# jack-nie/bitcoin-miner

Hardware: AMD Instinct MI355X
Metric: GH/s (SHA-256 nonce search) at 1/2/4/8 MI355X; % of VALU int roofline (higher is better)
Workload: dtype u32

## Files before the change

### bitcoin-miner_amd/csrc/minehip.cpp

```cpp
#include <hip/hip_runtime.h>
#include <stdlib.h>
#include <string.h>

#include <atomic>
#include <chrono>
#include <cmath>
#include <condition_variable>
#include <memory>
#include <mutex>
#include <string>
#include <system_error>
#include <thread>
#include <vector>

#include "../../include/minehip.h"
#include "../../include/minehip_server.h"
#include "layout.hpp"
#include "multi.hpp"
#include "plan.hpp"
#include "sched.hpp"

namespace mh {
hipError_t fast_module_init(int dev);
hipError_t launch_fast(int dev, int J, int mode, const FastArgs& a, Partial* partials, hipStream_t s);
hipError_t launch_generic_scan(const GenArgs& a, Partial* partials, uint32_t blocks, hipStream_t s);
hipError_t launch_hash_batch(const GenArgs& a, const uint64_t* d_nonces, uint64_t* d_out, uint64_t n,
                             hipStream_t s);
hipError_t launch_merge(const Partial* partials, uint32_t n, Partial* best, hipStream_t s);
}

namespace {

using mh::Partial;

thread_local std::string g_err;

int fail(int code, const std::string& what) {
    g_err = what;
    return code;
}

}

namespace mh {
int set_error(int code, const char* what) { return fail(code, what); }
}

namespace {

#define MH_HIP(call)                                                                                 \
    do {                                                                                             \
        hipError_t e_ = (call);                                                                      \
        if (e_ != hipSuccess) return fail(MH_EHIP, std::string(#call) + ": " + hipGetErrorString(e_)); \
    } while (0)

constexpr uint64_t kBatchChunk = 1u << 22;
constexpr int kEventPairs = 512;
constexpr uint32_t kQueueSlots = 4096;

struct Timed {
    hipEvent_t start = nullptr, stop = nullptr;
    int kind;
    int var;
};

struct VarStat {
    uint64_t launches = 0, nonces = 0, ns = 0, ops = 0, slots = 0;
};
constexpr int kVariants = 16 * mh::kModes * 5;
inline int var_index(int J, int mode, int L) { return J + 16 * mode + 16 * mh::kModes * (L - 1); }

struct DevCtx {
    std::mutex mu;
    int dev = -1;
    bool ready = false;
    hipStream_t stream = nullptr;
    hipStream_t ps[2] = {nullptr, nullptr};
    hipEvent_t ev_piece[2] = {nullptr, nullptr};
    hipEvent_t ev_main = nullptr;
    Partial* d_partials = nullptr;
    Partial* d_best = nullptr;
    Partial* h_best = nullptr;
    uint64_t* d_nonces = nullptr;
    uint64_t* d_hashes = nullptr;
    uint32_t poff = 0;
    uint32_t* d_counters = nullptr;
    uint32_t qoff = 0;
    bool prof = false;
    std::vector<Timed> pool;
    int used = 0;
    uint64_t cnt[8] = {0};
    VarStat var[kVariants];
};

std::mutex g_tab_mu;
std::vector<std::unique_ptr<DevCtx>> g_tab;
int g_ndev = -1;

int device_count_impl() {
    std::lock_guard<std::mutex> lk(g_tab_mu);
    if (g_ndev < 0) {
        int n = 0;
        if (hipGetDeviceCount(&n) != hipSuccess) n = 0;
        g_ndev = n;
        g_tab.resize((size_t)n);
        for (auto& p : g_tab) p.reset(new DevCtx());
    }
    return g_ndev;
}

int get_ctx(int dev, DevCtx** out) {
    const int n = device_count_impl();
    if (n <= 0) return fail(MH_ENODEV, "no HIP device visible");
    if (dev < 0 || dev >= n) return fail(MH_EINVAL, "device index out of range");
    DevCtx* c = g_tab[(size_t)dev].get();
    *out = c;
    return MH_OK;
}

int init_locked(DevCtx* c, int dev) {
    if (c->ready) return MH_OK;
    MH_HIP(hipSetDevice(dev));
    hipDeviceProp_t prop;
    MH_HIP(hipGetDeviceProperties(&prop, dev));
    if (strncmp(prop.gcnArchName, "gfx950", 6) != 0)
        return fail(MH_ENODEV, std::string("device is ") + prop.gcnArchName + ", kernels are built for gfx950 only");
    if (!c->stream) MH_HIP(hipStreamCreateWithFlags(&c->stream, hipStreamNonBlocking));
    if (!c->ps[0] || !c->ps[1]) {
        int least = 0, greatest = 0;
        MH_HIP(hipDeviceGetStreamPriorityRange(&least, &greatest));
        if (!c->ps[0]) MH_HIP(hipStreamCreateWithPriority(&c->ps[0], hipStreamNonBlocking, greatest));
        if (!c->ps[1]) MH_HIP(hipStreamCreateWithPriority(&c->ps[1], hipStreamNonBlocking, least));
    }
    for (auto& e : c->ev_piece)
        if (!e) MH_HIP(hipEventCreateWithFlags(&e, hipEventDisableTiming));
    if (!c->ev_main) MH_HIP(hipEventCreateWithFlags(&c->ev_main, hipEventDisableTiming));
    if (!c->d_partials) MH_HIP(hipMalloc(&c->d_partials, sizeof(Partial) * mh::kMaxBlocksPerLaunch));
    if (!c->d_best) MH_HIP(hipMalloc(&c->d_best, sizeof(Partial)));
    if (!c->d_counters) MH_HIP(hipMalloc(&c->d_counters, sizeof(uint32_t) * kQueueSlots));
    if (!c->h_best) MH_HIP(hipHostMalloc(&c->h_best, sizeof(Partial), hipHostMallocDefault));
    if (!c->d_nonces) MH_HIP(hipMalloc(&c->d_nonces, sizeof(uint64_t) * kBatchChunk));
    if (!c->d_hashes) MH_HIP(hipMalloc(&c->d_hashes, sizeof(uint64_t) * kBatchChunk));
    if (c->pool.empty()) c->pool.resize(kEventPairs);
    for (auto& t : c->pool) {
        if (!t.start) MH_HIP(hipEventCreate(&t.start));
        if (!t.stop) MH_HIP(hipEventCreate(&t.stop));
    }
    MH_HIP(mh::fast_module_init(dev));
    c->dev = dev;
    c->ready = true;
    return MH_OK;
}

int harvest_locked(DevCtx* c) {
    for (int i = 0; i < c->used; ++i) {
        float ms = 0.f;
        MH_HIP(hipEventElapsedTime(&ms, c->pool[(size_t)i].start, c->pool[(size_t)i].stop));
        const uint64_t ns = (uint64_t)((double)ms * 1.0e6);
        c->cnt[c->pool[(size_t)i].kind == 0 ? 2 : 5] += ns;
        if (c->pool[(size_t)i].kind == 0) c->var[c->pool[(size_t)i].var].ns += ns;
    }
    c->used = 0;
    return MH_OK;
}

int piece_streams_wait_main(DevCtx* c) {
    MH_HIP(hipEventRecord(c->ev_main, c->stream));
    for (auto s : c->ps) MH_HIP(hipStreamWaitEvent(s, c->ev_main, 0));
    return MH_OK;
}

int flush_partials(DevCtx* c, bool split) {
    if (!c->poff) return MH_OK;
    if (split) {
        for (int k = 0; k < 2; ++k) {
            MH_HIP(hipEventRecord(c->ev_piece[k], c->ps[k]));
            MH_HIP(hipStreamWaitEvent(c->stream, c->ev_piece[k], 0));
        }
    }
    MH_HIP(mh::launch_merge(c->d_partials, c->poff, c->d_best, c->stream));
    c->poff = 0;
    if (split) return piece_streams_wait_main(c);
    return MH_OK;
}

bool coarse_piece(const mh::Piece& p, const mh::PlanOpts& opt) { return p.kind == 0 && p.L == opt.lower_digits; }

bool early_piece_ok(const mh::Piece& p) {
    const mh::FastArgs& a = p.fa;
    const uint32_t J = (uint32_t)p.J;
    if ((a.inner >> 2) != J || a.hole + a.hole_w > a.n_hi + a.L) return false;
    for (uint32_t j = 0; j + 1u < a.L; ++j) {
        const uint32_t pos = a.g_last - j - (j >= a.g_hole ? 1u : 0u);
        if (pos > a.g_last || (pos >> 2) != J) return false;
    }
    return true;
}

int enqueue_piece(DevCtx* c, const mh::Piece& p, const mh::PlanOpts& opt, bool split) {
    hipStream_t s = !split ? c->stream : c->ps[coarse_piece(p, opt) ? 0 : 1];
    uint32_t blocks;
    if (p.kind == 0) {
        if (p.fa.n_runs == 0 || p.fa.L < 1 || p.fa.L > 5 || p.fa.n_hi + p.fa.L > 20)
            return fail(MH_EINTERNAL, "internal: bad fast piece");
        if (p.fa.mode >= mh::kModeOneEarly && !early_piece_ok(p))
            return fail(MH_EINTERNAL, "internal: bad Early piece (an enumerated digit outside word J)");
        blocks = (p.fa.n_runs + mh::kBlockThreads - 1) / mh::kBlockThreads;
    } else {
        if (p.ga.count == 0 || p.ga.count > (uint64_t)mh::kMaxBlocksPerLaunch * mh::kBlockThreads)
            return fail(MH_EINTERNAL, "internal: bad generic piece");
        blocks = (uint32_t)((p.ga.count + mh::kBlockThreads - 1) / mh::kBlockThreads);
    }
    if (blocks > mh::kMaxBlocksPerLaunch) return fail(MH_EINTERNAL, "internal: grid too large");
    if (c->poff + blocks > mh::kMaxBlocksPerLaunch) {
        const int rc = flush_partials(c, split);
        if (rc) return rc;
    }
    Partial* out = c->d_partials + c->poff;
    Timed* tm = nullptr;
    mh::FastArgs fa = p.fa;
    if (p.kind == 0) {
        fa.n_chunks = blocks;
        fa.counter = (opt.queue && c->qoff < kQueueSlots) ? c->d_counters + c->qoff++ : nullptr;
    }
    if (c->prof) {
        if (c->used == kEventPairs) {
            MH_HIP(hipStreamSynchronize(c->stream));
            for (auto ps : c->ps) MH_HIP(hipStreamSynchronize(ps));
            int rc = harvest_locked(c);
            if (rc) return rc;
        }
        tm = &c->pool[(size_t)c->used++];
        tm->kind = p.kind;
        tm->var = p.kind == 0 ? var_index(p.J, p.mode, p.L) : 0;
        MH_HIP(hipEventRecord(tm->start, s));
    }
    if (p.kind == 0)
        MH_HIP(mh::launch_fast(c->dev, p.J, p.mode, fa, out, s));
    else
        MH_HIP(mh::launch_generic_scan(p.ga, out, blocks, s));
    if (tm) MH_HIP(hipEventRecord(tm->stop, s));
    c->poff += blocks;
    if (c->prof) {
        if (p.kind == 0) {
            const uint64_t n = p.count;
            c->cnt[0] += 1;
            c->cnt[1] += n;
            c->cnt[3] += n * (uint64_t)p.ops;
            c->cnt[6] += n * (uint64_t)p.slots;
            VarStat& v = c->var[var_index(p.J, p.mode, p.L)];
            v.launches += 1;
            v.nonces += n;
            v.ops += n * (uint64_t)p.ops;
            v.slots += n * (uint64_t)p.slots;
        } else {
            c->cnt[4] += p.count;
        }
    }
    return MH_OK;
}

mh::PlanOpts plan_opts() {
    mh::PlanOpts o;
    if (const char* e = getenv("MINEHIP_LOWER_DIGITS")) {
        const int v = atoi(e);
        if (v >= 1 && v <= 5) o.lower_digits = v;
    }
    if (const char* e = getenv("MINEHIP_MIN_LANES")) o.min_lanes = strtoull(e, nullptr, 10);
    if (const char* e = getenv("MINEHIP_LAUNCH_NONCES")) {
        const unsigned long long v = strtoull(e, nullptr, 10);
        if (v >= 1) o.max_nonces_per_launch = v;
    }
    if (const char* e = getenv("MINEHIP_GENERIC_BELOW")) o.generic_below = strtoull(e, nullptr, 10);
    if (const char* e = getenv("MINEHIP_MAX_BLOCKS")) {
        const unsigned long long v = strtoull(e, nullptr, 10);
        if (v >= 1 && v <= mh::kMaxBlocksPerLaunch) o.max_blocks = (uint32_t)v;
    }
    if (const char* e = getenv("MINEHIP_STREAMS")) {
        const int v = atoi(e);
        if (v == 1 || v == 2) o.streams = v;
    }
    if (const char* e = getenv("MINEHIP_FINE_TAIL")) o.fine_tail = strtoull(e, nullptr, 10);
    if (const char* e = getenv("MINEHIP_QUEUE")) {
        const int v = atoi(e);
        if (v == 0 || v == 1) o.queue = v;
    }
    if (const char* e = getenv("MINEHIP_EARLY")) {
        const int v = atoi(e);
        if (v == 0 || v == 1) o.early = v;
    }
    return o;
}

uint64_t now_ns() {
    return (uint64_t)std::chrono::duration_cast<std::chrono::nanoseconds>(
               std::chrono::steady_clock::now().time_since_epoch())
        .count();
}

int search_impl(int dev, const mh::Prefix& pre, uint64_t lower, uint64_t upper, uint64_t* oh, uint64_t* on,
                uint64_t* busy_ns = nullptr) {
    DevCtx* c;
    int rc = get_ctx(dev, &c);
    if (rc) return rc;
    std::lock_guard<std::mutex> lk(c->mu);
    rc = init_locked(c, dev);
    if (rc) return rc;
    const uint64_t t0 = now_ns();
    MH_HIP(hipSetDevice(dev));
    MH_HIP(hipMemsetAsync(c->d_best, 0xFF, sizeof(Partial), c->stream));
    const mh::PlanOpts opt = plan_opts();
    if (opt.queue) MH_HIP(hipMemsetAsync(c->d_counters, 0, sizeof(uint32_t) * kQueueSlots, c->stream));
    c->qoff = 0;
    bool any_coarse = false, any_fine = false;
    if (opt.streams == 2)
        mh::plan_search(pre, lower, upper, opt, [&](const mh::Piece& p) {
            (coarse_piece(p, opt) ? any_coarse : any_fine) = true;
            return !(any_coarse && any_fine);
        });
    const bool split = opt.streams == 2 && any_coarse && any_fine;
    if (split) {
        rc = piece_streams_wait_main(c);
        if (rc) return rc;
    }
    int err = MH_OK;
    c->poff = 0;
    mh::plan_search(pre, lower, upper, opt, [&](const mh::Piece& p) {
        err = enqueue_piece(c, p, opt, split);
        return err == MH_OK;
    });
    if (!err) err = flush_partials(c, split);
    if (err) {
        for (auto ps : c->ps)
            if (ps) (void)hipStreamSynchronize(ps);
        (void)hipStreamSynchronize(c->stream);
        return err;
    }
    MH_HIP(hipMemcpyAsync(c->h_best, c->d_best, sizeof(Partial), hipMemcpyDeviceToHost, c->stream));
    MH_HIP(hipStreamSynchronize(c->stream));
    if (c->prof) {
        rc = harvest_locked(c);
        if (rc) return rc;
    }
    *oh = c->h_best->hash;
    *on = c->h_best->nonce;
    if (busy_ns) *busy_ns = now_ns() - t0;
    return MH_OK;
}

int check_common(const uint8_t* msg, size_t len) {
    if (msg == nullptr && len != 0) return fail(MH_EINVAL, "msg is NULL");
    if (len > MH_MAX_MSG_LEN) return fail(MH_ETOOLONG, "message longer than MH_MAX_MSG_LEN");
    return MH_OK;
}

}

extern "C" {

int mh_abi_version(void) { return MH_ABI_VERSION; }

int mh_device_count(void) { return device_count_impl(); }

const char* mh_last_error(void) { return g_err.c_str(); }

int mh_search(int dev, const uint8_t* msg, size_t len, uint64_t lower, uint64_t upper, uint64_t* out_hash,
              uint64_t* out_nonce) {
    g_err.clear();
    if (!out_hash || !out_nonce) return fail(MH_EINVAL, "NULL output pointer");
    int rc = check_common(msg, len);
    if (rc) return rc;
    if (lower > upper) return fail(MH_ERANGE, "lower > upper");
    mh::Prefix pre;
    mh::absorb_prefix(msg, len, &pre);
    return search_impl(dev, pre, lower, upper, out_hash, out_nonce);
}

int mh_search_multi(const int* devs, int ndev, const uint8_t* msg, size_t len, uint64_t lower, uint64_t upper,
                    uint64_t chunk, uint64_t* out_hash, uint64_t* out_nonce) {
    g_err.clear();
    if (!out_hash || !out_nonce || !devs || ndev <= 0) return fail(MH_EINVAL, "bad arguments");
    if (ndev > MH_MAX_WORKERS) return fail(MH_EINVAL, "more than MH_MAX_WORKERS devices listed");
    int rc = check_common(msg, len);
    if (rc) return rc;
    if (lower > upper) return fail(MH_ERANGE, "lower > upper");
    const int n = mh_device_count();
    for (int i = 0; i < ndev; ++i)
        if (devs[i] < 0 || devs[i] >= n) return fail(n <= 0 ? MH_ENODEV : MH_EINVAL, "device index out of range");
    mh::Prefix pre;
    mh::absorb_prefix(msg, len, &pre);
    int fail_worker = -1;
    mh::ThreadStart start;
#ifdef MH_DEV_HOOKS
    if (const char* e = getenv("MINEHIP_TEST_FAIL_WORKER")) fail_worker = atoi(e);
    if (const char* e = getenv("MINEHIP_TEST_SPAWN_LIMIT")) {
        auto started = std::make_shared<std::atomic<int>>(0);
        const int limit = atoi(e);
        start = [started, limit](std::function<void()> fn) {
            if ((*started)++ >= limit)
                throw std::system_error(std::make_error_code(std::errc::resource_unavailable_try_again));
            return std::thread(std::move(fn));
        };
    }
#endif
    if (ndev == 1 && chunk == 0 && fail_worker < 0 && !start)
        return search_impl(devs[0], pre, lower, upper, out_hash, out_nonce);
    if (chunk == 0) {
        const mh::SpanSearch search = [&](int worker, int dev, uint64_t lo, uint64_t hi, uint64_t* h, uint64_t* n,
                                          uint64_t* ns, std::string* err) {
            const int r = (worker == fail_worker) ? fail(MH_EHIP, "injected failure (dev build test hook)")
                                                  : search_impl(dev, pre, lo, hi, h, n, ns);
            if (r) *err = g_err;
            return r;
        };
        std::string err;
        const int r = mh::search_shards(devs, ndev, pre, lower, upper, plan_opts(), search, out_hash, out_nonce, &err,
                                        start);
        return r ? fail(r, err) : MH_OK;
    }
    const mh::ChunkSearch csearch = [&](int worker, uint64_t lo, uint64_t hi, uint64_t* h, uint64_t* nn,
                                        std::string* err) {
        const int r = (worker == fail_worker) ? fail(MH_EHIP, "injected failure (dev build test hook)")
                                              : search_impl(devs[worker], pre, lo, hi, h, nn);
        if (r) *err = g_err;
        return r;
    };
    std::string err;
    const int r = mh::search_chunks(ndev, msg, len, lower, upper, chunk, csearch, out_hash, out_nonce, &err, start);
    return r ? fail(r, err) : MH_OK;
}

int mh_hash_batch(int dev, const uint8_t* msg, size_t len, const uint64_t* nonces, size_t n, uint64_t* out_hashes) {
    g_err.clear();
    int rc = check_common(msg, len);
    if (rc) return rc;
    if (n == 0) return MH_OK;
    if (!nonces || !out_hashes) return fail(MH_EINVAL, "NULL buffer");
    DevCtx* c;
    rc = get_ctx(dev, &c);
    if (rc) return rc;
    std::lock_guard<std::mutex> lk(c->mu);
    rc = init_locked(c, dev);
    if (rc) return rc;
    MH_HIP(hipSetDevice(dev));
    mh::Prefix pre;
    mh::absorb_prefix(msg, len, &pre);
    mh::GenArgs ga;
    mh::make_gen_args(pre, &ga);
    for (size_t off = 0; off < n; off += kBatchChunk) {
        const size_t m = (n - off < kBatchChunk) ? n - off : kBatchChunk;
        MH_HIP(hipMemcpyAsync(c->d_nonces, nonces + off, m * sizeof(uint64_t), hipMemcpyHostToDevice, c->stream));
        MH_HIP(mh::launch_hash_batch(ga, c->d_nonces, c->d_hashes, m, c->stream));
        MH_HIP(hipMemcpyAsync(out_hashes + off, c->d_hashes, m * sizeof(uint64_t), hipMemcpyDeviceToHost, c->stream));
        MH_HIP(hipStreamSynchronize(c->stream));
    }
    return MH_OK;
}

int mh_profile_enable(int dev, int on) {
    g_err.clear();
    DevCtx* c;
    int rc = get_ctx(dev, &c);
    if (rc) return rc;
    std::lock_guard<std::mutex> lk(c->mu);
    rc = init_locked(c, dev);
    if (rc) return rc;
    MH_HIP(hipStreamSynchronize(c->stream));
    rc = harvest_locked(c);
    if (rc) return rc;
    if (on) {
        memset(c->cnt, 0, sizeof c->cnt);
        for (auto& v : c->var) v = VarStat();
    }
    c->prof = on != 0;
    return MH_OK;
}

int mh_profile_read(int dev, uint64_t* out, int n) {
    g_err.clear();
    if (!out || n < 0) return fail(MH_EINVAL, "bad arguments");
    DevCtx* c;
    int rc = get_ctx(dev, &c);
    if (rc) return rc;
    std::lock_guard<std::mutex> lk(c->mu);
    if (c->ready) {
        MH_HIP(hipStreamSynchronize(c->stream));
        rc = harvest_locked(c);
        if (rc) return rc;
    }
    for (int i = 0; i < n && i < 8; ++i) out[i] = c->cnt[i];
    return MH_OK;
}

int mh_profile_kernels(int dev, mh_kernel_stat* out, int cap) {
    g_err.clear();
    if (cap < 0 || (!out && cap > 0)) return fail(MH_EINVAL, "bad arguments");
    DevCtx* c;
    int rc = get_ctx(dev, &c);
    if (rc) return rc;
    std::lock_guard<std::mutex> lk(c->mu);
    if (c->ready) {
        MH_HIP(hipStreamSynchronize(c->stream));
        rc = harvest_locked(c);
        if (rc) return rc;
    }
    int n = 0;
    for (int i = 0; i < kVariants; ++i) {
        const VarStat& v = c->var[i];
        if (!v.launches) continue;
        if (n < cap) {
            out[n].word = i % 16;
            out[n].mode = (i / 16) % mh::kModes;
            out[n].lo_digits = i / (16 * mh::kModes) + 1;
            out[n].reserved = 0;
            out[n].launches = v.launches;
            out[n].nonces = v.nonces;
            out[n].ns = v.ns;
            out[n].ops = v.ops;
            out[n].slots = v.slots;
        }
        ++n;
    }
    return n;
}

int64_t mh_plan(const uint8_t* msg, size_t len, uint64_t lower, uint64_t upper, mh_piece* out, int64_t cap) {
    g_err.clear();
    int rc = check_common(msg, len);
    if (rc) return rc;
    if (lower > upper) return fail(MH_ERANGE, "lower > upper");
    if (cap < 0) return fail(MH_EINVAL, "cap < 0");
    mh::Prefix pre;
    mh::absorb_prefix(msg, len, &pre);
    int64_t k = 0;
    const mh::PlanOpts opt = plan_opts();
    mh::plan_search(pre, lower, upper, opt, [&](const mh::Piece& p) {
        if (k >= cap) {
            ++k;
            return false;
        }
        if (out) {
            mh_piece& q = out[k];
            q.first = p.first;
            q.count = p.count;
            q.kind = p.kind;
            q.digits = p.digits;
            q.lo_digits = p.L;
            q.word = p.J;
            q.mode = p.mode;
            q.blocks = p.blocks;
            q.nonce_ops = p.ops;
            q.nonce_slots = p.slots;
        }
        ++k;
        return true;
    });
    return k;
}

int64_t mh_multi_plan(const uint8_t* msg, size_t len, uint64_t lower, uint64_t upper, const double* weights,
                      int ndev, mh_span* out, int64_t cap) {
    g_err.clear();
    int rc = check_common(msg, len);
    if (rc) return rc;
    if (lower > upper) return fail(MH_ERANGE, "lower > upper");
    if (ndev <= 0 || ndev > MH_MAX_WORKERS || cap < 0) return fail(MH_EINVAL, "bad arguments");
    std::vector<double> w((size_t)ndev, 1.0);
    if (weights)
        for (int i = 0; i < ndev; ++i) {
            if (!(weights[i] > 0.0) || !std::isfinite(weights[i])) return fail(MH_EINVAL, "weights must be finite and > 0");
            w[(size_t)i] = weights[i];
        }
    mh::Prefix pre;
    mh::absorb_prefix(msg, len, &pre);
    mh::MultiPlan mp;
    mh::multi_plan(pre, lower, upper, plan_opts(), w, &mp);
    int64_t k = 0;
    auto put = [&](const mh::Span& s, int worker, int kind) {
        if (k < cap && out) {
            out[k].lower = s.lo;
            out[k].upper = s.hi;
            out[k].worker = worker;
            out[k].kind = kind;
            out[k].cost = mh::segments_cost(mp.segs, s.lo, s.hi);
        }
        ++k;
    };
    for (int i = 0; i < ndev; ++i)
        if (!mp.head[(size_t)i].empty) put(mp.head[(size_t)i], i, 0);
    for (const auto& s : mp.tail) put(s, -1, 1);
    return k;
}

int mh_multi_rates(const int* devs, int ndev, double* out) {
    g_err.clear();
    if (ndev < 0 || (ndev > 0 && (!devs || !out))) return fail(MH_EINVAL, "bad arguments");
    for (int i = 0; i < ndev; ++i) out[i] = mh::device_rate(devs[i]);
    return MH_OK;
}

}
```

### bitcoin-miner_amd/csrc/plan.cpp

```cpp
#include "plan.hpp"

#include <string.h>

#include <algorithm>
#include <cmath>

namespace mh {
namespace {

constexpr uint32_t kK[64] = {
    0x428a2f98u, 0x71374491u, 0xb5c0fbcfu, 0xe9b5dba5u, 0x3956c25bu, 0x59f111f1u, 0x923f82a4u, 0xab1c5ed5u,
    0xd807aa98u, 0x12835b01u, 0x243185beu, 0x550c7dc3u, 0x72be5d74u, 0x80deb1feu, 0x9bdc06a7u, 0xc19bf174u,
    0xe49b69c1u, 0xefbe4786u, 0x0fc19dc6u, 0x240ca1ccu, 0x2de92c6fu, 0x4a7484aau, 0x5cb0a9dcu, 0x76f988dau,
    0x983e5152u, 0xa831c66du, 0xb00327c8u, 0xbf597fc7u, 0xc6e00bf3u, 0xd5a79147u, 0x06ca6351u, 0x14292967u,
    0x27b70a85u, 0x2e1b2138u, 0x4d2c6dfcu, 0x53380d13u, 0x650a7354u, 0x766a0abbu, 0x81c2c92eu, 0x92722c85u,
    0xa2bfe8a1u, 0xa81a664bu, 0xc24b8b70u, 0xc76c51a3u, 0xd192e819u, 0xd6990624u, 0xf40e3585u, 0x106aa070u,
    0x19a4c116u, 0x1e376c08u, 0x2748774cu, 0x34b0bcb5u, 0x391c0cb3u, 0x4ed8aa4au, 0x5b9cca4fu, 0x682e6ff3u,
    0x748f82eeu, 0x78a5636fu, 0x84c87814u, 0x8cc70208u, 0x90befffau, 0xa4506cebu, 0xbef9a3f7u, 0xc67178f2u};
constexpr uint32_t kIV[8] = {0x6a09e667u, 0xbb67ae85u, 0x3c6ef372u, 0xa54ff53au,
                             0x510e527fu, 0x9b05688cu, 0x1f83d9abu, 0x5be0cd19u};

inline uint32_t ror(uint32_t x, int n) { return (x >> n) | (x << (32 - n)); }

constexpr uint64_t kPow10[20] = {1ull,
                                 10ull,
                                 100ull,
                                 1000ull,
                                 10000ull,
                                 100000ull,
                                 1000000ull,
                                 10000000ull,
                                 100000000ull,
                                 1000000000ull,
                                 10000000000ull,
                                 100000000000ull,
                                 1000000000000ull,
                                 10000000000000ull,
                                 100000000000000ull,
                                 1000000000000000ull,
                                 10000000000000000ull,
                                 100000000000000000ull,
                                 1000000000000000000ull,
                                 10000000000000000000ull};

inline void put_byte(uint32_t* w, uint32_t pos, uint32_t v) { w[pos >> 2] |= v << (24u - 8u * (pos & 3u)); }

void schedule(const uint32_t w16[16], uint32_t w[64]) {
    for (int i = 0; i < 16; ++i) w[i] = w16[i];
    for (int i = 16; i < 64; ++i) {
        const uint32_t s0 = ror(w[i - 15], 7) ^ ror(w[i - 15], 18) ^ (w[i - 15] >> 3);
        const uint32_t s1 = ror(w[i - 2], 17) ^ ror(w[i - 2], 19) ^ (w[i - 2] >> 10);
        w[i] = w[i - 16] + s0 + w[i - 7] + s1;
    }
}

}

int decimal_digits(uint64_t n) {
    int d = 1;
    while (d < 20 && n >= kPow10[d]) ++d;
    return d;
}

void host_compress(uint32_t st[8], const uint32_t w16[16]) {
    uint32_t w[64];
    schedule(w16, w);
    uint32_t a = st[0], b = st[1], c = st[2], d = st[3], e = st[4], f = st[5], g = st[6], h = st[7];
    for (int i = 0; i < 64; ++i) {
        const uint32_t t1 = h + (ror(e, 6) ^ ror(e, 11) ^ ror(e, 25)) + ((e & f) ^ (~e & g)) + kK[i] + w[i];
        const uint32_t t2 = (ror(a, 2) ^ ror(a, 13) ^ ror(a, 22)) + ((a & b) ^ (a & c) ^ (b & c));
        h = g; g = f; f = e; e = d + t1;
        d = c; c = b; b = a; a = t1 + t2;
    }
    st[0] += a; st[1] += b; st[2] += c; st[3] += d;
    st[4] += e; st[5] += f; st[6] += g; st[7] += h;
}

void absorb_prefix(const uint8_t* msg, size_t len, Prefix* out) {
    memcpy(out->mid, kIV, sizeof kIV);
    out->plen = (uint64_t)len + 1u;
    const uint64_t nfull = out->plen / 64u;
    uint32_t w[16];
    for (uint64_t blk = 0; blk < nfull; ++blk) {
        for (int i = 0; i < 16; ++i) {
            uint32_t v = 0;
            for (int k = 0; k < 4; ++k) {
                const uint64_t p = blk * 64u + (uint64_t)(4 * i + k);
                const uint32_t byte = (p < len) ? msg[p] : (uint32_t)' ';
                v = (v << 8) | byte;
            }
            w[i] = v;
        }
        host_compress(out->mid, w);
    }
    out->t = (uint32_t)(out->plen % 64u);
    memset(out->tail, 0, sizeof out->tail);
    for (uint32_t i = 0; i < out->t; ++i) {
        const uint64_t p = nfull * 64u + i;
        out->tail[i] = (p < len) ? msg[p] : (uint8_t)' ';
    }
}

void make_gen_args(const Prefix& pre, GenArgs* ga) {
    memset(ga, 0, sizeof *ga);
    memcpy(ga->mid, pre.mid, sizeof pre.mid);
    for (uint32_t i = 0; i < pre.t; ++i) put_byte(ga->tail, i, pre.tail[i]);
    ga->plen = pre.plen;
    ga->t = pre.t;
}

NonceCost nonce_cost(int J, int mode) {
    uint64_t dep = 1ull << J;
    for (int t = 16; t < 64; ++t)
        if (((dep >> (t - 2)) | (dep >> (t - 7)) | (dep >> (t - 15)) | (dep >> (t - 16))) & 1ull) dep |= 1ull << t;
    auto is = [&](int t) { return (dep >> t) & 1ull; };
    uint32_t ops = 0, slots = 0;
    for (int t = 16; t < 64; ++t) {
        if (!is(t)) continue;
        const int s0 = (int)is(t - 15), s1 = (int)is(t - 2), a16 = (int)is(t - 16), a7 = (int)is(t - 7);
        const int hoisted = (s0 && s1 && a16 && a7) ? 0 : 1;
        const int terms = s0 + s1 + a16 + a7 + hoisted;
        const bool x0 = s0 && t - 15 == J, x1 = s1 && t - 2 == J;
        ops += (uint32_t)((s0 ? (x0 ? 1 : 4) : 0) + (s1 ? (x1 ? 1 : 4) : 0)) + (uint32_t)terms / 2u;
        slots += (uint32_t)((s0 ? (x0 ? 1 : 6) : 0) + (s1 ? (x1 ? 1 : 6) : 0)) + (uint32_t)(terms - 1);
    }
    ops += 3u;
    slots += 3u;
    for (int t = J + 1; t < 64; ++t) {
        const bool inv_w = !is(t), inv_h = inv_w && t <= J + 3;
        ops += inv_h ? 13u : 14u;
        slots += 16u + (inv_h ? 5u : inv_w ? 6u : 7u);
    }
    if (mode % 3 == kModeTwo) {
        ops += 8u;
        slots += 8u;
        ops += 64u * 14u - 1u;
        slots += 64u * 22u - 1u;
    } else {
        ops -= 1u;
        slots -= 1u;
    }
    ops += 2u;
    slots += 2u;
    return NonceCost{ops, slots};
}

uint32_t nonce_ops(int J, int mode) { return nonce_cost(J, mode).ops; }

namespace {

bool kernel_exists(int J, int mode) { return fast_kernel_exists(J, mode); }

bool make_fast_args(const Prefix& pre, int d, int L, bool early, int* J_out, int* mode_out, int* blocks_out,
                    uint64_t* block_out, FastArgs* fa) {
    const uint32_t t = pre.t;
    const uint32_t total = t + (uint32_t)d;
    const int nb = (total + 9u <= 64u) ? 1 : 2;
    const uint32_t pl = total - 1u;
    int mode;
    uint32_t base;
    if (nb == 1) {
        mode = kModeOne;
        base = 0;
    } else if (pl >= 64u) {
        mode = kModePre;
        base = 64;
        if (!early && pl - (uint32_t)L + 1u < 64u) return false;
    } else {
        mode = kModeTwo;
        base = 0;
    }
    const uint32_t lo = pl - (uint32_t)L + 1u - base;
    int J = (int)((pl - base) >> 2);
    uint32_t p = 0, ib = 0;
    if (!early) {
        if ((int)(lo >> 2) < J - 1) return false;
    } else {
        if (J < 1) return false;
        ib = base + 4u * (uint32_t)J - 1u;
        if (ib < t || ib < base) return false;
        p = pl - ib;
        if (p < 1u || p >= (uint32_t)d) return false;
        if (L > 4 || p + (uint32_t)L > (uint32_t)d || ib - (uint32_t)(L - 1) < t || ib - (uint32_t)(L - 1) < base)
            return false;
        J -= 1;
        mode += 3;
    }
    if (!kernel_exists(J, mode)) return false;

    memset(fa, 0, sizeof *fa);
    memcpy(fa->mid, pre.mid, sizeof pre.mid);
    for (uint32_t i = 0; i < t; ++i) put_byte(fa->blk, i, pre.tail[i]);
    for (uint32_t i = 0; i < (uint32_t)d; ++i) put_byte(fa->blk, t + i, 0x30u);
    put_byte(fa->blk, total, 0x80u);
    const uint64_t bits = (pre.plen + (uint64_t)d) * 8u;
    const int lw = nb * 16 - 2;
    fa->blk[lw] = (uint32_t)(bits >> 32);
    fa->blk[lw + 1] = (uint32_t)bits;
    fa->pow10L = kPow10[L];
    fa->hi_end = total - (uint32_t)L;
    fa->n_hi = (uint32_t)(d - L);
    fa->lo_pos = lo;
    fa->L = (uint32_t)L;
    fa->n_groups = (uint32_t)kPow10[L - 1];
    fa->mode = (uint32_t)mode;
    fa->hole = kNoHole;
    fa->g_hole = kNoHole;
    fa->hole_w = 1;
    fa->g_mul = 1;
    uint64_t block = kPow10[L];
    if (early) {
        fa->inner = ib - base;
        fa->i_mul = kPow10[p];
        fa->g_last = ib - 1u - base;
        fa->hi_end = total;
        fa->hole = p;
        fa->hole_w = (uint32_t)L;
        fa->u_mul = 1;
        fa->g_mul = kPow10[p + 1u];
        block = kPow10[p + (uint32_t)L];
    }
    *block_out = block;
    if (mode % 3 == kModeTwo) {
        uint32_t w[64];
        schedule(fa->blk + 16, w);
        for (int i = 0; i < 64; ++i) fa->kw1[i] = kK[i] + w[i];
    }
    *J_out = J;
    *mode_out = mode;
    *blocks_out = nb;
    return true;
}

bool pick_layout(const Prefix& pre, int d, int L, uint64_t A, uint64_t B, const PlanOpts& opt, int* J, int* mode,
                 int* nb, uint64_t* block, FastArgs* fa) {
    if (!make_fast_args(pre, d, L, false, J, mode, nb, block, fa)) return false;
    if (opt.early) {
        int Je, me, nbe;
        uint64_t be;
        FastArgs fe;
        const uint64_t max_gen = (uint64_t)std::min(opt.max_blocks, kMaxBlocksPerLaunch) * kBlockThreads;
        if (make_fast_args(pre, d, L, true, &Je, &me, &nbe, &be, &fe) &&
            nonce_cost(Je, me).slots < nonce_cost(*J, *mode).slots && B - A >= 2u * be &&
            be <= opt.max_nonces_per_launch && be / kPow10[L] <= max_gen) {
            *J = Je;
            *mode = me;
            *nb = nbe;
            *block = be;
            *fa = fe;
        }
    }
    return true;
}

bool bucket_layout(const Prefix& pre, int d, uint64_t A, uint64_t B, const PlanOpts& opt, int* L_out, int* J,
                   int* mode, int* nb, uint64_t* block, FastArgs* fa) {
    int L = std::min(opt.lower_digits, d - 1);
    L = std::min(L, 5);
    while (L > 1 && (B - A) / kPow10[L] + 1u < opt.min_lanes) --L;
    while (L >= 1 && !pick_layout(pre, d, L, A, B, opt, J, mode, nb, block, fa)) --L;
    *L_out = L;
    return L >= 1 && B - A >= opt.generic_below;
}

inline uint64_t bucket_lo(int d) { return d == 1 ? 0u : kPow10[d - 1]; }
inline uint64_t bucket_hi(int d) { return d == 20 ? ~(uint64_t)0 : kPow10[d] - 1u; }

}

void cost_segments(const Prefix& pre, uint64_t lower, uint64_t upper, const PlanOpts& opt,
                   std::vector<CostSeg>* out) {
    out->clear();
    const int d_lo = decimal_digits(lower), d_hi = decimal_digits(upper);
    for (int d = d_lo; d <= d_hi; ++d) {
        const uint64_t A = std::max(lower, bucket_lo(d)), B = std::min(upper, bucket_hi(d));
        int L = 0, J = 0, mode = 0, nb = 1;
        uint64_t blk = 1;
        FastArgs fa;
        double per;
        bool steady = false;
        if (bucket_layout(pre, d, A, B, opt, &L, &J, &mode, &nb, &blk, &fa)) {
            steady = L == opt.lower_digits && (B - A) / kPow10[L] + 1u >= (1u << 21);
            per = (double)nonce_cost(J, mode).slots * (1.0 + 0.03 * (double)(3 - std::min(L, 3)));
            if (!steady) per *= kUnsteadyFactor;
        } else {
            const int blocks = (pre.t + (uint32_t)d + 9u <= 64u) ? 1 : 2;
            per = (double)kGenericSlotsPerBlock * blocks;
        }
        out->push_back(CostSeg{A, B, per, steady});
    }
}

double unsteady_share(const std::vector<CostSeg>& segs, uint64_t lo, uint64_t hi) {
    double all = 0.0, unsteady = 0.0;
    for (const CostSeg& s : segs) {
        const uint64_t a = std::max(s.a, lo), b = std::min(s.b, hi);
        if (a > b) continue;
        const double c = ((double)(b - a) + 1.0) * s.per;
        all += c;
        if (!s.steady) unsteady += c;
    }
    return all > 0.0 ? unsteady / all : 0.0;
}

double segments_cost(const std::vector<CostSeg>& segs, uint64_t lo, uint64_t hi) {
    double c = 0.0;
    for (const CostSeg& s : segs) {
        const uint64_t a = std::max(s.a, lo), b = std::min(s.b, hi);
        if (a <= b) c += ((double)(b - a) + 1.0) * s.per;
    }
    return c;
}

void split_by_cost(const std::vector<CostSeg>& segs, const std::vector<double>& w, std::vector<Span>* out) {
    out->assign(w.size(), Span{0, 0, true});
    if (segs.empty() || w.empty()) return;
    using u128 = unsigned __int128;
    double wsum = 0.0;
    for (double x : w) wsum += std::max(0.0, x);
    double total = 0.0;
    for (const CostSeg& s : segs) total += ((double)(s.b - s.a) + 1.0) * s.per;
    const uint64_t lower = segs.front().a;
    const u128 n_all = (u128)(segs.back().b - lower) + 1u;
    u128 prev = 0;
    double acc_w = 0.0;
    for (size_t k = 0; k < w.size(); ++k) {
        acc_w += std::max(0.0, w[k]);
        u128 pos;
        if (k + 1 == w.size() || wsum <= 0.0) {
            pos = (k + 1 == w.size()) ? n_all : prev;
        } else {
            double target = total * (acc_w / wsum), cum = 0.0;
            pos = n_all;
            for (const CostSeg& s : segs) {
                const double len = (double)(s.b - s.a) + 1.0, c = len * s.per;
                if (cum + c >= target) {
                    double n = std::floor((target - cum) / s.per);
                    n = std::min(std::max(n, 0.0), len);
                    pos = (u128)(s.a - lower) + (u128)n;
                    break;
                }
                cum += c;
            }
            if (pos > n_all) pos = n_all;
        }
        if (pos < prev) pos = prev;
        if (pos > prev) (*out)[k] = Span{(uint64_t)(lower + (prev)), (uint64_t)(lower + (pos - 1u)), false};
        prev = pos;
    }
}

void plan_search(const Prefix& pre, uint64_t lower, uint64_t upper, const PlanOpts& opt,
                 const std::function<bool(const Piece&)>& cb) {
    GenArgs gbase;
    make_gen_args(pre, &gbase);
    const int d_lo = decimal_digits(lower), d_hi = decimal_digits(upper);
    const uint64_t max_gen = (uint64_t)std::min(opt.max_blocks, kMaxBlocksPerLaunch) * kBlockThreads;

    bool have_gen = false;
    uint64_t gen_a = 0, gen_b = 0;
    auto flush_generic = [&]() -> bool {
        if (!have_gen) return true;
        have_gen = false;
        Piece p;
        memset(&p, 0, sizeof p);
        p.first = gen_a;
        p.count = gen_b - gen_a + 1u;
        p.kind = 1;
        p.digits = decimal_digits(gen_a);
        p.blocks = ((pre.t + (uint32_t)decimal_digits(gen_b) + 9u) <= 64u) ? 1 : 2;
        p.ga = gbase;
        p.ga.first = gen_a;
        p.ga.count = p.count;
        return cb(p);
    };
    auto emit_generic = [&](uint64_t a, uint64_t b, int) -> bool {
        for (;;) {
            if (have_gen && gen_b - gen_a < max_gen - 1u && gen_b + 1u == a) {
                const uint64_t room = max_gen - 1u - (gen_b - gen_a);
                if (b - a < room) {
                    gen_b = b;
                    return true;
                }
                gen_b = a + (room - 1u);
                a = gen_b + 1u;
            }
            if (!flush_generic()) return false;
            const uint64_t left = b - a;
            const uint64_t cnt = (left >= max_gen - 1u) ? max_gen : left + 1u;
            have_gen = true;
            gen_a = a;
            gen_b = a + (cnt - 1u);
            if (cnt - 1u == left) return true;
            a += cnt;
        }
    };

    auto emit_runs = [&](int d, unsigned __int128 ua, unsigned __int128 ub, uint64_t Bx, int Lx, int Jx, int modex,
                         int nbx, const FastArgs& fax) -> bool {
        const unsigned __int128 Rx = kPow10[Lx];
        const uint64_t lpb = Bx / (uint64_t)Rx;
        uint64_t max_runs = std::min<uint64_t>(max_gen, opt.max_nonces_per_launch / (uint64_t)Rx);
        max_runs = std::max<uint64_t>(lpb, max_runs / lpb * lpb);
        ua *= lpb;
        ub *= lpb;
        for (unsigned __int128 u = ua; u < ub;) {
            const unsigned __int128 left = ub - u;
            const uint64_t runs = (left > max_runs) ? max_runs : (uint64_t)left;
            Piece p;
            memset(&p, 0, sizeof p);
            p.first = (uint64_t)(u * Rx);
            p.count = (uint64_t)((unsigned __int128)runs * Rx);
            p.kind = 0;
            p.digits = d;
            p.L = Lx;
            p.J = Jx;
            p.mode = modex;
            p.blocks = nbx;
            p.fa = fax;
            { const NonceCost nc = nonce_cost(Jx, modex); p.ops = nc.ops; p.slots = nc.slots; }
            p.fa.u_start = (uint64_t)u;
            p.fa.n_runs = (uint32_t)runs;
            p.ga = gbase;
            if (!flush_generic() || !cb(p)) return false;
            u += runs;
        }
        return true;
    };
    auto emit_edge = [&](int d, uint64_t a, uint64_t b) -> bool {
        FastArgs fs;
        int Js = 0, ms = 0, nbs = 1;
        uint64_t bs = 1;
        const int L = 1;
        if (!make_fast_args(pre, d, L, false, &Js, &ms, &nbs, &bs, &fs)) return emit_generic(a, b, d);
        const unsigned __int128 R = bs;
        const unsigned __int128 u0 = ((unsigned __int128)a + R - 1u) / R, u1 = ((unsigned __int128)b + 1u) / R;
        if (u0 >= u1) return emit_generic(a, b, d);
        if (a < (uint64_t)(u0 * R) && !emit_generic(a, (uint64_t)(u0 * R) - 1u, d)) return false;
        if (!emit_runs(d, u0, u1, bs, L, Js, ms, nbs, fs)) return false;
        return u1 * R > (unsigned __int128)b || emit_generic((uint64_t)(u1 * R), b, d);
    };

    for (int d = d_lo; d <= d_hi; ++d) {
        const uint64_t A = std::max(lower, bucket_lo(d)), B = std::min(upper, bucket_hi(d));
        FastArgs fa;
        int L = 0, J = 0, mode = 0, nb = 1;
        uint64_t blk = 1;
        if (!bucket_layout(pre, d, A, B, opt, &L, &J, &mode, &nb, &blk, &fa)) {
            if (!emit_generic(A, B, d)) return;
            continue;
        }
        const bool early = mode >= 3;
        const unsigned __int128 R = blk;
        const unsigned __int128 U0 = ((unsigned __int128)A + R - 1u) / R;
        const unsigned __int128 U1p = ((unsigned __int128)B + 1u) / R;
        if (U0 >= U1p) {
            if (!(early ? emit_edge(d, A, B) : emit_generic(A, B, d))) return;
            continue;
        }
        const uint64_t fast_first = (uint64_t)(U0 * R);
        const unsigned __int128 fast_end = U1p * R;
        if (A < fast_first && !(early ? emit_edge(d, A, fast_first - 1u) : emit_generic(A, fast_first - 1u, d)))
            return;
        unsigned __int128 U_split = U1p;
        int Lf = 0, Jf = 0, modef = 0, nbf = 1;
        uint64_t blkf = 1;
        FastArgs faf;
        if (opt.fine_tail && L == opt.lower_digits && L >= 2) {
            const unsigned __int128 tail_blocks = opt.fine_tail / (uint64_t)R;
            if (tail_blocks >= 1 && (U1p - U0) > 4 * tail_blocks &&
                pick_layout(pre, d, L - 1, A, B, opt, &Jf, &modef, &nbf, &blkf, &faf) && R % blkf == 0u) {
                U_split = U1p - tail_blocks;
                Lf = L - 1;
            }
        }
        if (!emit_runs(d, U0, U_split, blk, L, J, mode, nb, fa)) return;
        if (U_split < U1p && !emit_runs(d, U_split * (R / blkf), U1p * (R / blkf), blkf, Lf, Jf, modef, nbf, faf))
            return;
        if (fast_end <= (unsigned __int128)B &&
            !(early ? emit_edge(d, (uint64_t)fast_end, B) : emit_generic((uint64_t)fast_end, B, d)))
            return;
    }
    flush_generic();
}

}
```

### bitcoin-miner_amd/csrc/plan.hpp

```cpp
#pragma once
#include <stdint.h>
#include <stddef.h>

#include <functional>
#include <vector>

#include "layout.hpp"

namespace mh {

struct Prefix {
    uint32_t mid[8];
    uint8_t tail[64];
    uint32_t t;
    uint64_t plen;
};

void absorb_prefix(const uint8_t* msg, size_t len, Prefix* out);

void host_compress(uint32_t st[8], const uint32_t w16[16]);

struct Piece {
    uint64_t first;
    uint64_t count;
    int kind;
    int digits;
    int L;
    int J;
    int mode;
    int blocks;
    uint32_t ops;
    uint32_t slots;
    FastArgs fa;
    GenArgs ga;
};

struct PlanOpts {
    int lower_digits = 3;
    uint64_t min_lanes = 1u << 19;
    uint64_t max_nonces_per_launch = 1ull << 35;
    uint32_t max_blocks = 1u << 17;
    uint64_t generic_below = 1u << 20;
    int streams = 2;
    uint64_t fine_tail = 1ull << 28;
    int queue = 1;
    int early = 1;
};

void plan_search(const Prefix& pre, uint64_t lower, uint64_t upper, const PlanOpts& opt,
                 const std::function<bool(const Piece&)>& cb);

void make_gen_args(const Prefix& pre, GenArgs* ga);

uint32_t nonce_ops(int J, int mode);

struct NonceCost {
    uint32_t ops, slots;
};
NonceCost nonce_cost(int J, int mode);

int decimal_digits(uint64_t n);

struct CostSeg {
    uint64_t a, b;
    double per;
    bool steady;
};
double unsteady_share(const std::vector<CostSeg>& segs, uint64_t lo, uint64_t hi);
constexpr double kGenericSlotsPerBlock = 2.0 * 1760.0;
constexpr double kUnsteadyFactor = 1.15;
void cost_segments(const Prefix& pre, uint64_t lower, uint64_t upper, const PlanOpts& opt,
                   std::vector<CostSeg>* out);
double segments_cost(const std::vector<CostSeg>& segs, uint64_t lo, uint64_t hi);

struct Span {
    uint64_t lo, hi;
    bool empty;
};
void split_by_cost(const std::vector<CostSeg>& segs, const std::vector<double>& w, std::vector<Span>* out);

}
```

Before: 54.42.

## Add third priority stream and optional coarse-piece lane ordering

Creates a third medium-priority piece stream and lets coarse pieces alternate between the high and medium streams when MINEHIP_COARSE_LANES=2. It also buffers the first 64 pieces so that, with MINEHIP_COARSE_FIRST=1, the largest coarse piece is enqueued first. The aim is better overlap and load balance between long and short kernels across streams. By default lane assignment is unchanged, but flushes now sync three streams and early enqueue is delayed by the prefix buffering.

```diff
diff --git a/bitcoin-miner_amd/csrc/minehip.cpp b/bitcoin-miner_amd/csrc/minehip.cpp
--- a/bitcoin-miner_amd/csrc/minehip.cpp
+++ b/bitcoin-miner_amd/csrc/minehip.cpp
@@ -75,8 +75,8 @@
     int dev = -1;
     bool ready = false;
     hipStream_t stream = nullptr;
-    hipStream_t ps[2] = {nullptr, nullptr};
-    hipEvent_t ev_piece[2] = {nullptr, nullptr};
+    hipStream_t ps[3] = {nullptr, nullptr, nullptr};
+    hipEvent_t ev_piece[3] = {nullptr, nullptr, nullptr};
     hipEvent_t ev_main = nullptr;
     Partial* d_partials = nullptr;
     Partial* d_best = nullptr;
@@ -126,11 +126,12 @@
     if (strncmp(prop.gcnArchName, "gfx950", 6) != 0)
         return fail(MH_ENODEV, std::string("device is ") + prop.gcnArchName + ", kernels are built for gfx950 only");
     if (!c->stream) MH_HIP(hipStreamCreateWithFlags(&c->stream, hipStreamNonBlocking));
-    if (!c->ps[0] || !c->ps[1]) {
+    if (!c->ps[0] || !c->ps[1] || !c->ps[2]) {
         int least = 0, greatest = 0;
         MH_HIP(hipDeviceGetStreamPriorityRange(&least, &greatest));
-        if (!c->ps[0]) MH_HIP(hipStreamCreateWithPriority(&c->ps[0], hipStreamNonBlocking, greatest));
-        if (!c->ps[1]) MH_HIP(hipStreamCreateWithPriority(&c->ps[1], hipStreamNonBlocking, least));
+        const int prio[3] = {greatest, (least + greatest) / 2, least};
+        for (int k = 0; k < 3; ++k)
+            if (!c->ps[k]) MH_HIP(hipStreamCreateWithPriority(&c->ps[k], hipStreamNonBlocking, prio[k]));
     }
     for (auto& e : c->ev_piece)
         if (!e) MH_HIP(hipEventCreateWithFlags(&e, hipEventDisableTiming));
@@ -173,7 +174,7 @@
 int flush_partials(DevCtx* c, bool split) {
     if (!c->poff) return MH_OK;
     if (split) {
-        for (int k = 0; k < 2; ++k) {
+        for (int k = 0; k < 3; ++k) {
             MH_HIP(hipEventRecord(c->ev_piece[k], c->ps[k]));
             MH_HIP(hipStreamWaitEvent(c->stream, c->ev_piece[k], 0));
         }
@@ -197,8 +198,9 @@
     return true;
 }
 
-int enqueue_piece(DevCtx* c, const mh::Piece& p, const mh::PlanOpts& opt, bool split) {
-    hipStream_t s = !split ? c->stream : c->ps[coarse_piece(p, opt) ? 0 : 1];
+int enqueue_piece(DevCtx* c, const mh::Piece& p, const mh::PlanOpts& opt, int lane) {
+    const bool split = lane >= 0;
+    hipStream_t s = split ? c->ps[lane] : c->stream;
     uint32_t blocks;
     if (p.kind == 0) {
         if (p.fa.n_runs == 0 || p.fa.L < 1 || p.fa.L > 5 || p.fa.n_hi + p.fa.L > 20)
@@ -289,6 +291,14 @@
         const int v = atoi(e);
         if (v == 0 || v == 1) o.early = v;
     }
+    if (const char* e = getenv("MINEHIP_COARSE_LANES")) {
+        const int v = atoi(e);
+        if (v == 1 || v == 2) o.coarse_lanes = v;
+    }
+    if (const char* e = getenv("MINEHIP_COARSE_FIRST")) {
+        const int v = atoi(e);
+        if (v == 0 || v == 1) o.coarse_first = v;
+    }
     return o;
 }
 
@@ -312,23 +322,52 @@
     const mh::PlanOpts opt = plan_opts();
     if (opt.queue) MH_HIP(hipMemsetAsync(c->d_counters, 0, sizeof(uint32_t) * kQueueSlots, c->stream));
     c->qoff = 0;
-    bool any_coarse = false, any_fine = false;
+    int n_coarse = 0;
+    bool any_fine = false, split = false;
     if (opt.streams == 2)
         mh::plan_search(pre, lower, upper, opt, [&](const mh::Piece& p) {
-            (coarse_piece(p, opt) ? any_coarse : any_fine) = true;
-            return !(any_coarse && any_fine);
+            if (coarse_piece(p, opt))
+                ++n_coarse;
+            else
+                any_fine = true;
+            split = (n_coarse >= 1 && any_fine) || (opt.coarse_lanes == 2 && n_coarse >= 2);
+            return !split;
         });
-    const bool split = opt.streams == 2 && any_coarse && any_fine;
     if (split) {
         rc = piece_streams_wait_main(c);
         if (rc) return rc;
     }
     int err = MH_OK;
     c->poff = 0;
+    std::vector<mh::Piece> prefix;
+    bool prefix_open = split;
+    int next_lane = mh::kLaneHigh;
+    const auto enqueue_prefix = [&]() {
+        std::vector<mh::LaneKey> keys;
+        for (const mh::Piece& p : prefix) keys.push_back({coarse_piece(p, opt), p.count});
+        std::vector<mh::LaneSlot> order;
+        mh::order_lanes(keys, opt.coarse_lanes, opt.coarse_first != 0, &next_lane, &order);
+        for (const mh::LaneSlot& o : order) {
+            err = enqueue_piece(c, prefix[o.piece], opt, o.lane);
+            if (err) break;
+        }
+        prefix.clear();
+        prefix_open = false;
+    };
     mh::plan_search(pre, lower, upper, opt, [&](const mh::Piece& p) {
-        err = enqueue_piece(c, p, opt, split);
+        if (prefix_open) {
+            prefix.push_back(p);
+            if (prefix.size() == mh::kLanePrefix) enqueue_prefix();
+        } else if (!split) {
+            err = enqueue_piece(c, p, opt, -1);
+        } else {
+            err = enqueue_piece(c, p, opt,
+                                coarse_piece(p, opt) ? mh::next_coarse_lane(opt.coarse_lanes, &next_lane)
+                                                     : (int)mh::kLaneLow);
+        }
         return err == MH_OK;
     });
+    if (!err && prefix_open) enqueue_prefix();
     if (!err) err = flush_partials(c, split);
     if (err) {
         for (auto ps : c->ps)
diff --git a/bitcoin-miner_amd/csrc/plan.cpp b/bitcoin-miner_amd/csrc/plan.cpp
--- a/bitcoin-miner_amd/csrc/plan.cpp
+++ b/bitcoin-miner_amd/csrc/plan.cpp
@@ -484,4 +484,18 @@
     flush_generic();
 }
 
-}
+void order_lanes(const std::vector<LaneKey>& prefix, int coarse_lanes, bool coarse_first, int* next,
+                 std::vector<LaneSlot>* out) {
+    out->clear();
+    out->reserve(prefix.size());
+    size_t lead = prefix.size();
+    if (coarse_first)
+        for (size_t i = 0; i < prefix.size(); ++i)
+            if (prefix[i].coarse && (lead == prefix.size() || prefix[i].count > prefix[lead].count)) lead = i;
+    if (lead < prefix.size()) out->push_back({(uint32_t)lead, next_coarse_lane(coarse_lanes, next)});
+    for (size_t i = 0; i < prefix.size(); ++i)
+        if (i != lead)
+            out->push_back({(uint32_t)i, prefix[i].coarse ? next_coarse_lane(coarse_lanes, next) : (int)kLaneLow});
+}
+
+}
diff --git a/bitcoin-miner_amd/csrc/plan.hpp b/bitcoin-miner_amd/csrc/plan.hpp
--- a/bitcoin-miner_amd/csrc/plan.hpp
+++ b/bitcoin-miner_amd/csrc/plan.hpp
@@ -45,10 +45,30 @@
     uint64_t fine_tail = 1ull << 28;
     int queue = 1;
     int early = 1;
+    int coarse_lanes = 1;
+    int coarse_first = 0;
 };
 
 void plan_search(const Prefix& pre, uint64_t lower, uint64_t upper, const PlanOpts& opt,
                  const std::function<bool(const Piece&)>& cb);
+
+enum Lane { kLaneHigh = 0, kLaneNormal = 1, kLaneLow = 2 };
+constexpr size_t kLanePrefix = 64;
+struct LaneKey {
+    bool coarse;
+    uint64_t count;
+};
+struct LaneSlot {
+    uint32_t piece;
+    int lane;
+};
+inline int next_coarse_lane(int coarse_lanes, int* next) {
+    const int lane = *next;
+    if (coarse_lanes == 2) *next = lane == kLaneHigh ? kLaneNormal : kLaneHigh;
+    return lane;
+}
+void order_lanes(const std::vector<LaneKey>& prefix, int coarse_lanes, bool coarse_first, int* next,
+                 std::vector<LaneSlot>* out);
 
 void make_gen_args(const Prefix& pre, GenArgs* ga);
 
```

After: 54.44, median of 2. Within noise of the previous version (+0.0%).
